# AIRI-Institute/nablaDFT

Measured on NVIDIA H100. Metric: molecules/sec (PaiNN E+F fwd+bwd), higher is better.
Workload: dtype f32

## Files before the change

nabladft_b200/csrc/painn_fused.cu:

```cuda
#include "painn_node.cuh"

#include "tc_pipe.cuh"

namespace {

constexpr int TILES_PER_LAYER = 22;

enum { T_UV = 0, T_UW, T_B1A, T_B1B, T_B2_0, T_B2_1, T_B2_2, T_A1, T_A2_0, T_A2_1, T_A2_2,
       T_B2T_0, T_B2T_1, T_B2T_2, T_B1AT, T_B1BT, T_UT_0, T_UT_1, T_A2T_0, T_A2T_1, T_A2T_2, T_A1T };

struct TileSrc { const float* p; int ld, row0, k0, trans, rows, kvalid; };

__device__ __forceinline__ TileSrc tile_src(const nb200_painn_weights& w, int idx) {
    const int L = w.n_layers;
    TileSrc s{nullptr, F, 0, 0, 0, 128, 128};
    if (idx >= L * TILES_PER_LAYER) {
        s.p = w.R1; s.ld = F;
        if (idx - L * TILES_PER_LAYER == 0) { s.rows = F / 2; } else { s.trans = 1; s.kvalid = F / 2; }
        return s;
    }
    const int l = idx / TILES_PER_LAYER, t = idx % TILES_PER_LAYER;
    const float* A1 = w.A1 + (size_t)l * F * F;
    const float* A2 = w.A2 + (size_t)l * 3 * F * F;
    const float* U = w.U + (size_t)l * 2 * F * F;
    const float* B1 = w.B1 + (size_t)l * F * 2 * F;
    const float* B2 = w.B2 + (size_t)l * 3 * F * F;
    switch (t) {
        case T_UV: s.p = U; break;
        case T_UW: s.p = U; s.row0 = F; break;
        case T_B1A: s.p = B1; s.ld = 2 * F; break;
        case T_B1B: s.p = B1; s.ld = 2 * F; s.k0 = F; break;
        case T_B2_0: case T_B2_1: case T_B2_2: s.p = B2; s.row0 = (t - T_B2_0) * F; break;
        case T_A1: s.p = A1; break;
        case T_A2_0: case T_A2_1: case T_A2_2: s.p = A2; s.row0 = (t - T_A2_0) * F; break;
        case T_B2T_0: case T_B2T_1: case T_B2T_2: s.p = B2; s.trans = 1; s.k0 = (t - T_B2T_0) * F; break;
        case T_B1AT: s.p = B1; s.ld = 2 * F; s.trans = 1; break;
        case T_B1BT: s.p = B1; s.ld = 2 * F; s.trans = 1; s.row0 = F; break;
        case T_UT_0: case T_UT_1: s.p = U; s.trans = 1; s.k0 = (t - T_UT_0) * F; break;
        case T_A2T_0: case T_A2T_1: case T_A2T_2: s.p = A2; s.trans = 1; s.k0 = (t - T_A2T_0) * F; break;
        default: s.p = A1; s.trans = 1; break;
    }
    return s;
}

__global__ void __launch_bounds__(256) k_prep_painn(nb200_painn_weights w, unsigned char* __restrict__ dst) {
    const int idx = blockIdx.x >> 2, st = blockIdx.x & 3;
    const TileSrc s = tile_src(w, idx);
    unsigned char* tile = dst + (size_t)idx * WTILE_BYTES;
#pragma unroll
    for (int i = 0; i < 4; ++i) {
        const int item = threadIdx.x + 256 * i;
        int kc, r;
        if (!s.trans) { kc = item & 7; r = item >> 3; } else { r = item & 127; kc = item >> 7; }
        const int k = st * 32 + kc * 4;
        float e[4];
#pragma unroll
        for (int j = 0; j < 4; ++j) {
            const bool ok = r < s.rows && k + j < s.kvalid;
            e[j] = !ok ? 0.f : !s.trans ? __ldg(s.p + (size_t)(s.row0 + r) * s.ld + s.k0 + k + j) : __ldg(s.p + (size_t)(s.k0 + k + j) * s.ld + s.row0 + r);
        }
        float4 hi, lo;
        split4(make_float4(e[0], e[1], e[2], e[3]), hi, lo);
        const int kk = 32 * st + 4 * kc;
        float* out_hi = reinterpret_cast<float*>(tile + (size_t)(kk / KSTAGE) * WST_BYTES + (size_t)((kk % KSTAGE) / 4) * WLBO) + r * 4;
        st4(out_hi, hi);
        st4(out_hi + (KSTAGE / 4) * WLBO / 4, lo);
    }
}

struct FwdParams {
    int xsplit;
    int n_atoms, do_upd, do_mlp, do_ro;
    const unsigned char* wt;
    int tile_upd, tile_mlp, tile_ro;
    const float *q_mid, *mu_mid, *d1, *d2;
    float *VW, *nrm, *dot, *g1pre, *y, *q_next, *mu_next;
    float eps;
    const float *q_mlp_in, *c1;
    float *h1pre, *xh;
    float* ro_pre;
};

__global__ void __launch_bounds__(NTHREADS, CTAS_PER_SM) k_node_fwd(const FwdParams P) {
    extern __shared__ __align__(1024) unsigned char smem[];
    __shared__ Prog prog;
    const int tid = threadIdx.x, warp = tid >> 5, lane = tid & 31;
    if (tid == 0) {
        prog.n = 0;
        if (P.do_upd) {
            for (int x = 0; x < 3; ++x) {
                prog_add(prog, P.tile_upd + T_UV, U_NEWX | U_FIRST | U_LAST);
                prog_add(prog, P.tile_upd + T_UW, U_FIRST | U_LAST | U_XLAST);
            }
            prog_add(prog, P.tile_upd + T_B1A, U_NEWX | U_FIRST | U_LAST | U_XLAST);
            prog_add(prog, P.tile_upd + T_B1B, U_NEWX | U_FIRST | U_LAST | U_XLAST);
            prog_add(prog, P.tile_upd + T_B2_1, U_NEWX | U_FIRST | U_LAST);
            prog_add(prog, P.tile_upd + T_B2_0, U_FIRST | U_LAST);
            prog_add(prog, P.tile_upd + T_B2_2, U_FIRST | U_LAST | U_XLAST);
        }
        if (P.do_mlp) {
            prog_add(prog, P.tile_mlp + T_A1, U_NEWX | U_FIRST | U_LAST | U_XLAST);
            prog_add(prog, P.tile_mlp + T_A2_0, U_NEWX | U_FIRST | U_LAST);
            prog_add(prog, P.tile_mlp + T_A2_1, U_FIRST | U_LAST);
            prog_add(prog, P.tile_mlp + T_A2_2, U_FIRST | U_LAST | U_XLAST);
        }
        if (P.do_ro) prog_add(prog, P.tile_ro, U_NEWX | U_FIRST | U_LAST | U_XLAST);
    }
    Ctx c = setup(smem, tid, P.xsplit);
    NF_PROF_DO(const long long tk0_ = clock64(); c.t_last = tk0_;)
#define NF_BASE 0

    if (warp >= WARP_ISSUE) {
        run_issuer(c, prog, P.wt);
        NF_PROF_DO(if (warp == WARP_ISSUE && lane == 0) { atomicAdd(&g_nf_prof[0], (unsigned long long)(clock64() - tk0_)); atomicAdd(&g_nf_prof[1], (unsigned long long)c.w_x);
                   atomicAdd(&g_nf_prof[2], (unsigned long long)c.w_buf); atomicAdd(&g_nf_prof[3], (unsigned long long)c.w_full); })
    } else {
        const int N = P.n_atoms, A0 = blockIdx.x * NT;
        const int fl = 32 * (warp & 3) + lane;
        const int n0 = CPT * (warp >> 2);
        const bool isE = role_epi(warp), isL = role_load(warp);
        const int ltid = load_tid(tid);
#define NF_LOAD(...) do { if (isL) load_x(c, ltid, __VA_ARGS__); else ++c.xg; } while (0)
        if (P.do_upd) {
#pragma unroll 1
            for (int x = 0; x < 3; ++x) {
                NF_LOAD([&](int r, int kc) { return A0 + r < N ? ldg4(P.mu_mid + (size_t)(A0 + r) * (3 * F) + x * F + 4 * kc) : f4(0.f); });
                NF_MARK(0);
#pragma unroll 1
                for (int half = 0; half < 2 && isE; ++half) {
                    drain(c, warp);
                    NF_MARK(1);
                    epi_chunks(c, warp, [&](int cb, float (&v)[16]) {
                        float* dst = P.VW + (size_t)(A0 + n0 + 16 * cb) * (6 * F) + x * 2 * F + half * F + fl;
#pragma unroll
                        for (int j = 0; j < 16; ++j)
                            if (A0 + n0 + 16 * cb + j < N) dst[(size_t)j * (6 * F)] = v[j];
                    });
                    NF_MARK(21);
                }
            }
            NF_MARK(2);
            if (isE) dep_signal(c, 0);
            NF_LOAD([&](int r, int kc) { return A0 + r < N ? ldg4(P.q_mid + (size_t)(A0 + r) * F + 4 * kc) : f4(0.f); });
            NF_MARK(3);
            if (isL) {
                dep_wait(c, 0);
                const int kc = ltid & 31, w = ltid >> 5;
#pragma unroll 1
                for (int it0 = 0; it0 < RPT; it0 += 2) {
                    float4 V[2][3], Wv[2][3];
#pragma unroll
                    for (int b = 0; b < 2; ++b) {
                        const int a = A0 + w + NLOAD * (it0 + b);
                        const float* vv = P.VW + (size_t)min(a, N - 1) * (6 * F) + 4 * kc;
#pragma unroll
                        for (int x = 0; x < 3; ++x) { V[b][x] = ld4(vv + x * 2 * F); Wv[b][x] = ld4(vv + x * 2 * F + F); }
                    }
#pragma unroll
                    for (int b = 0; b < 2; ++b) {
                        const int a = A0 + w + NLOAD * (it0 + b);
                        if (a < N) {
                            float4 sq = V[b][0] * V[b][0]; fma4(sq, V[b][1], V[b][1]); fma4(sq, V[b][2], V[b][2]);
                            float4 dt = f4(0.f); fma4(dt, V[b][0], Wv[b][0]); fma4(dt, V[b][1], Wv[b][1]); fma4(dt, V[b][2], Wv[b][2]);
                            st4(P.nrm + (size_t)a * F + 4 * kc, make_float4(sqrtf(sq.x + P.eps), sqrtf(sq.y + P.eps), sqrtf(sq.z + P.eps), sqrtf(sq.w + P.eps)));
                            st4(P.dot + (size_t)a * F + 4 * kc, dt);
                        }
                    }
                }
            }
            NF_MARK(4);
            if (isL) dep_signal(c, 1);
            NF_LOAD([&](int r, int kc) { return A0 + r < N ? ld4(P.nrm + (size_t)(A0 + r) * F + 4 * kc) : f4(0.f); });
            NF_MARK(5);
            if (isE) drain(c, warp);
            NF_MARK(6);
            NF_MARK(7);
            if (!isE) ++c.xg;
            else {
                drain(c, warp, 1);
                NF_MARK(8);
                const float b = __ldg(P.d1 + fl);
                const XPut xp(c, fl);
                epi_chunks(c, warp, [&](int cb, float (&v)[16]) {
#pragma unroll
                    for (int j = 0; j < 16; ++j) xp.put(n0 + 16 * cb + j, A0 + n0 + 16 * cb + j < N ? siluf_(v[j] + b) : 0.f);
                });
                xp.done(c);
                epi_chunks(c, warp, [&](int cb, float (&v)[16]) {
                    float* g = P.g1pre + (size_t)(A0 + n0 + 16 * cb) * F + fl;
#pragma unroll
                    for (int j = 0; j < 16; ++j)
                        if (A0 + n0 + 16 * cb + j < N) g[(size_t)j * F] = v[j] + b;
                });
            }
            NF_MARK(9);
            if (isE) {
                drain(c, warp);
                NF_MARK(10);
                const float b = __ldg(P.d2 + F + fl);
#pragma unroll 1
                for (int cb = 0; cb < CPT / 8; ++cb) {
                    float v16[16];
                    stage_ld16(c, warp, cb >> 1, v16);
                    float tw[8][3], tm[8][3];
#pragma unroll
                    for (int jj = 0; jj < 8; ++jj) {
                        const int a = min(A0 + n0 + 8 * cb + jj, N - 1);
                        const float* vw = P.VW + (size_t)a * (6 * F) + F + fl;
                        const float* mm = P.mu_mid + (size_t)a * (3 * F) + fl;
#pragma unroll
                        for (int x = 0; x < 3; ++x) { tw[jj][x] = vw[x * 2 * F]; tm[jj][x] = __ldg(mm + x * F); }
                    }
#pragma unroll
                    for (int jj = 0; jj < 8; ++jj) {
                        const int a = A0 + n0 + 8 * cb + jj;
                        if (a < N) {
                            const float y1 = ((cb & 1) ? v16[8 + jj] : v16[jj]) + b;
                            P.y[(size_t)a * (3 * F) + F + fl] = y1;
                            float* mo = P.mu_next + (size_t)a * (3 * F) + fl;
#pragma unroll
                            for (int x = 0; x < 3; ++x) mo[x * F] = fmaf(y1, tw[jj][x], tm[jj][x]);
                        }
                    }
                }
            }
            NF_MARK(11);
            if (isE) {
                drain(c, warp);
                NF_MARK(12);
                const float b = __ldg(P.d2 + fl);
                epi_chunks(c, warp, [&](int cb, float (&v)[16]) {
                    float t[16];
#pragma unroll
                    for (int j = 0; j < 16; ++j) t[j] = __ldg(P.q_mid + (size_t)min(A0 + n0 + 16 * cb + j, N - 1) * F + fl);
#pragma unroll
                    for (int j = 0; j < 16; ++j) {
                        const int a = A0 + n0 + 16 * cb + j;
                        if (a < N) {
                            const float y0 = v[j] + b;
                            P.y[(size_t)a * (3 * F) + fl] = y0;
                            P.q_next[(size_t)a * F + fl] = t[j] + y0;
                        }
                    }
                });
            }
            NF_MARK(13);
            if (!isE) ++c.xg;
            else {
                dep_wait(c, 1);
                drain(c, warp);
                NF_MARK(14);
                const float b = __ldg(P.d2 + 2 * F + fl);
                const XPut xp(c, fl);
                epi_chunks(c, warp, [&](int cb, float (&v)[16]) {
                    float tq[16], td[16];
#pragma unroll
                    for (int j = 0; j < 16; ++j) {
                        const size_t a = (size_t)min(A0 + n0 + 16 * cb + j, N - 1);
                        tq[j] = P.q_next[a * F + fl];
                        td[j] = P.dot[a * F + fl];
                    }
#pragma unroll
                    for (int j = 0; j < 16; ++j) {
                        const int a = A0 + n0 + 16 * cb + j;
                        float qn = 0.f;
                        if (a < N) {
                            qn = fmaf(v[j] + b, td[j], tq[j]);
                            P.q_next[(size_t)a * F + fl] = qn;
                        }
                        xp.put(n0 + 16 * cb + j, qn);
                    }
                });
                xp.done(c);
                epi_chunks(c, warp, [&](int cb, float (&v)[16]) {
#pragma unroll
                    for (int j = 0; j < 16; ++j)
                        if (A0 + n0 + 16 * cb + j < N) P.y[(size_t)(A0 + n0 + 16 * cb + j) * (3 * F) + 2 * F + fl] = v[j] + b;
                });
            }
        } else {
            NF_LOAD([&](int r, int kc) { return A0 + r < N ? ldg4(P.q_mlp_in + (size_t)(A0 + r) * F + 4 * kc) : f4(0.f); });
        }
        NF_MARK(15);
        if (P.do_mlp && !isE) ++c.xg;
        if (P.do_mlp && isE) {
            {
                drain(c, warp);
                NF_MARK(16);
                const float b = __ldg(P.c1 + fl);
                const XPut xp(c, fl);
                epi_chunks(c, warp, [&](int cb, float (&v)[16]) {
#pragma unroll
                    for (int j = 0; j < 16; ++j) xp.put(n0 + 16 * cb + j, siluf_(v[j] + b));
                });
                xp.done(c);
                epi_chunks(c, warp, [&](int cb, float (&v)[16]) {
#pragma unroll
                    for (int j = 0; j < 16; ++j)
                        if (A0 + n0 + 16 * cb + j < N) P.h1pre[(size_t)(A0 + n0 + 16 * cb + j) * F + fl] = v[j] + b;
                });
            }
            NF_MARK(17);
#pragma unroll 1
            for (int ct = 0; ct < 3; ++ct) {
                drain(c, warp);
                NF_MARK(18);
                epi_chunks(c, warp, [&](int cb, float (&v)[16]) {
                    float* dst = P.xh + (size_t)(A0 + n0 + 16 * cb) * (3 * F) + ct * F + fl;
#pragma unroll
                    for (int j = 0; j < 16; ++j)
                        if (A0 + n0 + 16 * cb + j < N) dst[(size_t)j * (3 * F)] = v[j];
                });
            }
        }
        NF_MARK(19);
        if (P.do_ro && isE) {
            drain(c, warp);
            epi_chunks(c, warp, [&](int cb, float (&v)[16]) {
                if (fl < F / 2) {
                    float* dst = P.ro_pre + (size_t)(A0 + n0 + 16 * cb) * (F / 2) + fl;
#pragma unroll
                    for (int j = 0; j < 16; ++j)
                        if (A0 + n0 + 16 * cb + j < N) dst[(size_t)j * (F / 2)] = v[j];
                }
            });
        }
#undef NF_LOAD
    }
    NF_MARK(20);
#undef NF_BASE
    NF_PROF_DO(if (tid == 0) { atomicAdd(&g_nf_prof[4], (unsigned long long)(clock64() - tk0_)); atomicAdd(&g_nf_prof[5], (unsigned long long)c.w_acc);
                            atomicAdd(&g_nf_prof[6], (unsigned long long)c.w_xfree); atomicAdd(&g_nf_prof[7], 1ull); })
}

struct BwdParams {
    int xsplit;
    int n_atoms, do_mlp, do_ro, do_upd;
    const unsigned char* wt;
    int tile_mlp, tile_ro, tile_upd;
    float *gq_a, *gq_b, *cur, *gn, *gdot;
    const float *g_xh, *h1pre, *dot;
    const float *ro_pre, *R2;
    const float *y, *VW, *nrm, *g1pre;
};

__global__ void __launch_bounds__(NTHREADS, CTAS_PER_SM) k_node_bwd(const BwdParams P) {
    extern __shared__ __align__(1024) unsigned char smem[];
    __shared__ Prog prog;
    const int tid = threadIdx.x, warp = tid >> 5, lane = tid & 31;
    if (tid == 0) {
        prog.n = 0;
        if (P.do_mlp) {
            prog_add(prog, P.tile_mlp + T_A2T_0, U_NEWX | U_FIRST | U_XLAST);
            prog_add(prog, P.tile_mlp + T_A2T_1, U_NEWX | U_XLAST);
            prog_add(prog, P.tile_mlp + T_A2T_2, U_NEWX | U_XLAST | U_LAST);
            prog_add(prog, P.tile_mlp + T_A1T, U_NEWX | U_FIRST | U_LAST | U_XLAST);
        } else if (P.do_ro) {
            prog_add(prog, P.tile_ro, U_NEWX | U_FIRST | U_LAST | U_XLAST);
        }
        if (P.do_upd) {
            prog_add(prog, P.tile_upd + T_B2T_0, U_NEWX | U_FIRST | U_XLAST);
            prog_add(prog, P.tile_upd + T_B2T_1, U_NEWX | U_XLAST);
            prog_add(prog, P.tile_upd + T_B2T_2, U_NEWX | U_XLAST | U_LAST);
            prog_add(prog, P.tile_upd + T_B1AT, U_NEWX | U_FIRST | U_LAST);
            prog_add(prog, P.tile_upd + T_B1BT, U_FIRST | U_LAST | U_XLAST);
            for (int x = 0; x < 3; ++x) {
                prog_add(prog, P.tile_upd + T_UT_0, U_NEWX | U_FIRST | U_XLAST);
                prog_add(prog, P.tile_upd + T_UT_1, U_NEWX | U_XLAST | U_LAST);
            }
        }
    }
    Ctx c = setup(smem, tid, P.xsplit);
    NF_PROF_DO(const long long tk0_ = clock64();)

    if (warp >= WARP_ISSUE) {
        run_issuer(c, prog, P.wt);
        NF_PROF_DO(if (warp == WARP_ISSUE && lane == 0) { atomicAdd(&g_nf_prof[8], (unsigned long long)(clock64() - tk0_)); atomicAdd(&g_nf_prof[9], (unsigned long long)c.w_x);
                   atomicAdd(&g_nf_prof[10], (unsigned long long)c.w_buf); atomicAdd(&g_nf_prof[11], (unsigned long long)c.w_full); })
    } else {
        const int N = P.n_atoms, A0 = blockIdx.x * NT;
        const int fl = 32 * (warp & 3) + lane;
        const int n0 = CPT * (warp >> 2);
        const bool isE = role_epi(warp), isL = role_load(warp);
        const int ltid = load_tid(tid);
#define NF_LOAD(...) do { if (isL) load_x(c, ltid, __VA_ARGS__); else ++c.xg; } while (0)
        if (P.do_mlp) {
#pragma unroll 1
            for (int ck = 0; ck < 3; ++ck)
                NF_LOAD([&](int r, int kc) { return A0 + r < N ? ldg4(P.g_xh + (size_t)(A0 + r) * (3 * F) + ck * F + 4 * kc) : f4(0.f); });
            if (!isE) ++c.xg;
            else {
                drain(c, warp);
                const XPut xp(c, fl);
                epi_chunks(c, warp, [&](int cb, float (&v)[16]) {
                    float t[16];
#pragma unroll
                    for (int j = 0; j < 16; ++j) t[j] = __ldg(P.h1pre + (size_t)min(A0 + n0 + 16 * cb + j, N - 1) * F + fl);
#pragma unroll
                    for (int j = 0; j < 16; ++j) xp.put(n0 + 16 * cb + j, A0 + n0 + 16 * cb + j < N ? v[j] * dsiluf_(t[j]) : 0.f);
                });
                xp.done(c);
            }
        } else if (P.do_ro) {
            NF_LOAD([&](int r, int kc) {
                if (A0 + r >= N || kc >= F / 8) return f4(0.f);
                const float4 p = ldg4(P.ro_pre + (size_t)(A0 + r) * (F / 2) + 4 * kc), w2 = ldg4(P.R2 + 4 * kc);
                return make_float4(w2.x * dsiluf_(p.x), w2.y * dsiluf_(p.y), w2.z * dsiluf_(p.z), w2.w * dsiluf_(p.w));
            });
        }
        if ((P.do_mlp || P.do_ro) && isE) {
            drain(c, warp);
            epi_chunks(c, warp, [&](int cb, float (&v)[16]) {
                float t[16], ty[16];
#pragma unroll
                for (int j = 0; j < 16; ++j) {
                    const size_t a = (size_t)min(A0 + n0 + 16 * cb + j, N - 1);
                    t[j] = P.do_mlp ? P.gq_a[a * F + fl] : 0.f;
                    ty[j] = P.do_upd ? __ldg(P.y + a * (3 * F) + 2 * F + fl) : 0.f;
                }
#pragma unroll
                for (int j = 0; j < 16; ++j) {
                    const int a = A0 + n0 + 16 * cb + j;
                    if (a < N) {
                        const float g = t[j] + v[j];
                        P.gq_b[(size_t)a * F + fl] = g;
                        if (P.do_upd) P.gdot[(size_t)a * F + fl] = g * ty[j];
                    }
                }
            });
        }
        if (P.do_upd) {
            if (isE) dep_signal(c, 0);
            if (isL) dep_wait(c, 0);
            NF_LOAD([&](int r, int kc) { return A0 + r < N ? ld4(P.gq_b + (size_t)(A0 + r) * F + 4 * kc) : f4(0.f); });
            NF_LOAD([&](int r, int kc) {
                if (A0 + r >= N) return f4(0.f);
                const float* vw = P.VW + (size_t)(A0 + r) * (6 * F) + F + 4 * kc;
                const float* gm = P.cur + (size_t)(A0 + r) * (3 * F) + 4 * kc;
                float4 sacc = f4(0.f);
#pragma unroll
                for (int x = 0; x < 3; ++x) fma4(sacc, ld4(gm + x * F), ldg4(vw + x * 2 * F));
                return sacc;
            });
            NF_LOAD([&](int r, int kc) {
                return A0 + r < N ? ld4(P.gq_b + (size_t)(A0 + r) * F + 4 * kc) * ldg4(P.dot + (size_t)(A0 + r) * F + 4 * kc) : f4(0.f);
            });
            if (!isE) ++c.xg;
            else {
                drain(c, warp);
                const XPut xp(c, fl);
                epi_chunks(c, warp, [&](int cb, float (&v)[16]) {
                    float t[16];
#pragma unroll
                    for (int j = 0; j < 16; ++j) t[j] = __ldg(P.g1pre + (size_t)min(A0 + n0 + 16 * cb + j, N - 1) * F + fl);
#pragma unroll
                    for (int j = 0; j < 16; ++j) xp.put(n0 + 16 * cb + j, A0 + n0 + 16 * cb + j < N ? v[j] * dsiluf_(t[j]) : 0.f);
                });
                xp.done(c);
            }
            if (isE) {
                drain(c, warp);
                epi_chunks(c, warp, [&](int cb, float (&v)[16]) {
                    float t[16];
#pragma unroll
                    for (int j = 0; j < 16; ++j) t[j] = P.gq_b[(size_t)min(A0 + n0 + 16 * cb + j, N - 1) * F + fl];
#pragma unroll
                    for (int j = 0; j < 16; ++j)
                        if (A0 + n0 + 16 * cb + j < N) P.gq_a[(size_t)(A0 + n0 + 16 * cb + j) * F + fl] = t[j] + v[j];
                });
            }
            if (isE) {
                drain(c, warp);
                epi_chunks(c, warp, [&](int cb, float (&v)[16]) {
                    float t[16];
#pragma unroll
                    for (int j = 0; j < 16; ++j) t[j] = __ldg(P.nrm + (size_t)min(A0 + n0 + 16 * cb + j, N - 1) * F + fl);
#pragma unroll
                    for (int j = 0; j < 16; ++j)
                        if (A0 + n0 + 16 * cb + j < N) P.gn[(size_t)(A0 + n0 + 16 * cb + j) * F + fl] = v[j] / t[j];
                });
            }
            if (isE) dep_signal(c, 1);
            if (isL) dep_wait(c, 1);
#pragma unroll 1
            for (int x = 0; x < 3; ++x) {
                NF_LOAD([&](int r, int kc) {
                    if (A0 + r >= N) return f4(0.f);
                    const size_t a = (size_t)(A0 + r);
                    float4 o = ld4(P.gdot + a * F + 4 * kc) * ldg4(P.VW + a * (6 * F) + x * 2 * F + F + 4 * kc);
                    fma4(o, ld4(P.gn + a * F + 4 * kc), ldg4(P.VW + a * (6 * F) + x * 2 * F + 4 * kc));
                    return o;
                });
                NF_LOAD([&](int r, int kc) {
                    if (A0 + r >= N) return f4(0.f);
                    const size_t a = (size_t)(A0 + r);
                    float4 o = ld4(P.cur + a * (3 * F) + x * F + 4 * kc) * ldg4(P.y + a * (3 * F) + F + 4 * kc);
                    fma4(o, ld4(P.gdot + a * F + 4 * kc), ldg4(P.VW + a * (6 * F) + x * 2 * F + 4 * kc));
                    return o;
                });
                if (isE) {
                drain(c, warp);
                epi_chunks(c, warp, [&](int cb, float (&v)[16]) {
                    float t[16];
#pragma unroll
                    for (int j = 0; j < 16; ++j) t[j] = P.cur[(size_t)min(A0 + n0 + 16 * cb + j, N - 1) * (3 * F) + x * F + fl];
#pragma unroll
                    for (int j = 0; j < 16; ++j)
                        if (A0 + n0 + 16 * cb + j < N) P.cur[(size_t)(A0 + n0 + 16 * cb + j) * (3 * F) + x * F + fl] = t[j] + v[j];
                });
                }
            }
        }
#undef NF_LOAD
    }
    NF_PROF_DO(if (tid == 0) { atomicAdd(&g_nf_prof[12], (unsigned long long)(clock64() - tk0_)); atomicAdd(&g_nf_prof[13], (unsigned long long)c.w_acc);
                            atomicAdd(&g_nf_prof[14], (unsigned long long)c.w_xfree); atomicAdd(&g_nf_prof[15], 1ull); })
}

template <class K>
int set_smem(K kernel) {
    return cudaFuncSetAttribute(kernel, cudaFuncAttributeMaxDynamicSharedMemorySize, SMEM_TOTAL) == cudaSuccess ? NB200_OK : nb_check_launch();
}

}

#ifdef NF_PROF
extern "C" int nb200_debug_nf_prof(unsigned long long* out16, int reset) {
    if (cudaMemcpyFromSymbol(out16, g_nf_prof, sizeof(unsigned long long) * 16) != cudaSuccess) return -1;
    if (reset) { unsigned long long z[16] = {0}; cudaMemcpyToSymbol(g_nf_prof, z, sizeof(z)); }
    return 0;
}
extern "C" int nb200_debug_nf_phase(unsigned long long* out64, int reset) {
    if (cudaMemcpyFromSymbol(out64, g_nf_phase, sizeof(unsigned long long) * 64) != cudaSuccess) return -1;
    if (reset) { unsigned long long z[64] = {0}; cudaMemcpyToSymbol(g_nf_phase, z, sizeof(z)); }
    return 0;
}
#endif

int64_t nb_fused_wtile_bytes(int n_layers) { return (int64_t)(n_layers * TILES_PER_LAYER + 2) * WTILE_BYTES; }

int nb_fused_prep(const nb200_painn_weights* w, void* wtiles, cudaStream_t s) {
    const int n_tiles = w->n_layers * TILES_PER_LAYER + 2;
    k_prep_painn<<<n_tiles * 4, 256, 0, s>>>(*w, static_cast<unsigned char*>(wtiles));
    return nb_check_launch();
}

static int nf_xsplit() {
    static const int on = [] { const char* e = getenv("NB200_NF_XSPLIT"); return (e && e[0] == '1') ? 1 : 0; }();
    return on;
}

int nb_fused_node_fwd(const NbFusedFwd& a, cudaStream_t s) {
    static bool attr = false;
    if (!attr) { if (set_smem(k_node_fwd) != NB200_OK) return NB200_ECUDA; attr = true; }
    FwdParams P{};
    P.xsplit = nf_xsplit();
    P.n_atoms = a.n_atoms; P.do_upd = a.layer_upd >= 0; P.do_mlp = a.layer_mlp >= 0; P.do_ro = a.readout;
    P.wt = static_cast<const unsigned char*>(a.wtiles);
    P.tile_upd = a.layer_upd * TILES_PER_LAYER; P.tile_mlp = a.layer_mlp * TILES_PER_LAYER; P.tile_ro = a.n_layers * TILES_PER_LAYER;
    P.q_mid = a.q_mid; P.mu_mid = a.mu_mid; P.d1 = a.d1; P.d2 = a.d2; P.VW = a.VW; P.nrm = a.nrm; P.dot = a.dot; P.g1pre = a.g1pre; P.y = a.y;
    P.q_next = a.q_next; P.mu_next = a.mu_next; P.eps = a.eps; P.q_mlp_in = a.q_mlp_in; P.c1 = a.c1; P.h1pre = a.h1pre; P.xh = a.xh;
    P.ro_pre = a.ro_pre;
    if (a.n_atoms <= 0) return NB200_OK;
    k_node_fwd<<<(a.n_atoms + NT - 1) / NT, NTHREADS, SMEM_TOTAL, s>>>(P);
    return nb_check_launch();
}

int nb_fused_node_bwd(const NbFusedBwd& a, cudaStream_t s) {
    static bool attr = false;
    if (!attr) { if (set_smem(k_node_bwd) != NB200_OK) return NB200_ECUDA; attr = true; }
    BwdParams P{};
    P.xsplit = nf_xsplit();
    P.n_atoms = a.n_atoms; P.do_mlp = a.layer_mlp >= 0; P.do_ro = a.readout; P.do_upd = a.layer_upd >= 0;
    P.wt = static_cast<const unsigned char*>(a.wtiles);
    P.tile_mlp = a.layer_mlp * TILES_PER_LAYER; P.tile_ro = a.n_layers * TILES_PER_LAYER + 1; P.tile_upd = a.layer_upd * TILES_PER_LAYER;
    P.gq_a = a.gq_a; P.gq_b = a.gq_b; P.cur = a.cur; P.gn = a.gn; P.gdot = a.gdot; P.dot = a.dot; P.g_xh = a.g_xh; P.h1pre = a.h1pre; P.ro_pre = a.ro_pre; P.R2 = a.R2;
    P.y = a.y; P.VW = a.VW; P.nrm = a.nrm; P.g1pre = a.g1pre;
    if (a.n_atoms <= 0) return NB200_OK;
    k_node_bwd<<<(a.n_atoms + NT - 1) / NT, NTHREADS, SMEM_TOTAL, s>>>(P);
    return nb_check_launch();
}
```

nabladft_b200/csrc/tc_pipe.cuh:

```cuda
#pragma once
#include "common.cuh"
#include "wgmma.cuh"

namespace {


constexpr int F = NB_F;
constexpr int NT = 64, KSTAGE = 32, W_STAGES = 3, NWORK = 8, CTAS_PER_SM = 1;
constexpr int XLBO = NT * 16 + 16;
constexpr int XLBOF = XLBO / 4;
constexpr int X_BYTES = 32 * XLBO;
constexpr int WLBO = 128 * 16;
constexpr int WST_BYTES = 2 * (KSTAGE / 4) * WLBO;
constexpr int STAGES_PER_TILE = 128 / KSTAGE;
constexpr int WTILE_BYTES = STAGES_PER_TILE * WST_BYTES;
constexpr int SROW = NT + 4;
constexpr int STAGE_BYTES = 128 * SROW * 4;
constexpr int SMEM_BARS = 2 * X_BYTES + W_STAGES * WST_BYTES + STAGE_BYTES;
constexpr int SMEM_TOTAL = SMEM_BARS + 256;
static_assert(SMEM_TOTAL <= 227 * 1024, "shared memory of one CTA");
#ifdef NF_TWO_GROUPS
constexpr int NEPI = NWORK / 2, NLOAD = NWORK / 2;
#else
constexpr int NEPI = NWORK, NLOAD = NWORK;
#endif
constexpr int CPT = NT / (NEPI / 4);
constexpr int RPT = NT / NLOAD;
constexpr int WARP_ISSUE = NWORK;
constexpr int NTHREADS = 32 * (NWORK + 8);
static_assert(NWORK % 4 == 0, "the MMA warpgroups must start on a warpgroup boundary");
enum { U_NEWX = 1, U_FIRST = 2, U_LAST = 4, U_XLAST = 8 };
#ifdef NF_PROF
__device__ unsigned long long g_nf_prof[16];
__device__ unsigned long long g_nf_phase[64];
#define NF_PROF_DO(...) __VA_ARGS__
#define NF_MARK(i) do { if (tid == 0) { const long long now_ = clock64(); atomicAdd(&g_nf_phase[NF_BASE + (i)], (unsigned long long)(now_ - c.t_last)); c.t_last = now_; } } while (0)
#else
#define NF_PROF_DO(...)
#define NF_MARK(i)
#endif

struct Prog {
    int n;
    uint16_t tile[24];
    uint8_t flag[24];
};

__device__ __forceinline__ uint32_t s_u32(const void* p) { return (uint32_t)__cvta_generic_to_shared(p); }
__device__ __forceinline__ void mbar_init(uint64_t* bar, uint32_t count) {
    asm volatile("mbarrier.init.shared::cta.b64 [%0], %1;" ::"r"(s_u32(bar)), "r"(count) : "memory");
}
__device__ __forceinline__ void mbar_wait(uint64_t* bar, uint32_t parity) {
    asm volatile(
        "{\n.reg .pred P1;\nLAB_WAIT:\nmbarrier.try_wait.parity.shared::cta.b64 P1, [%0], %1;\n@P1 bra DONE;\nbra LAB_WAIT;\nDONE:\n}\n" ::"r"(
            s_u32(bar)),
        "r"(parity)
        : "memory");
}
__device__ __forceinline__ void mbar_arrive(uint64_t* bar) { asm volatile("mbarrier.arrive.shared::cta.b64 _, [%0];" ::"r"(s_u32(bar)) : "memory"); }
__device__ __forceinline__ void mbar_expect_tx(uint64_t* bar, uint32_t bytes) {
    asm volatile("mbarrier.arrive.expect_tx.shared::cta.b64 _, [%0], %1;" ::"r"(s_u32(bar)), "r"(bytes) : "memory");
}
__device__ __forceinline__ void bulk_g2s(void* dst, const void* src, uint32_t bytes, uint64_t* bar) {
    asm volatile("cp.async.bulk.shared::cluster.global.mbarrier::complete_tx::bytes [%0], [%1], %2, [%3];" ::"r"(s_u32(dst)), "l"(src), "r"(bytes),
                 "r"(s_u32(bar))
                 : "memory");
}
__device__ __forceinline__ float tf32_rn(float x) {
    uint32_t r;
    asm("cvt.rna.tf32.f32 %0, %1;" : "=r"(r) : "f"(x));
    return __uint_as_float(r);
}
__device__ __forceinline__ void split_tf32(float x, float& hi, float& lo) {
    hi = tf32_rn(x);
    lo = tf32_rn(x - hi);
}
__device__ __forceinline__ void split4(const float4 v, float4& hi, float4& lo) {
    split_tf32(v.x, hi.x, lo.x); split_tf32(v.y, hi.y, lo.y); split_tf32(v.z, hi.z, lo.z); split_tf32(v.w, hi.w, lo.w);
}
__device__ __forceinline__ void work_barrier() { asm volatile("bar.sync 1, %0;" ::"n"(32 * NWORK) : "memory"); }
__device__ __forceinline__ float4 ld4(const float* p) { return *reinterpret_cast<const float4*>(p); }

struct Ctx {
    float *x_hi, *x_lo;
    unsigned char* ring;
    float* stage;
    uint64_t *full, *empty, *x_ready, *x_free, *acc_full, *stage_free, *dep;
    uint64_t *x_ready2, *x_free2;
    int xsplit = 0;
    int xg = 0;
    int o = 0;
    NF_PROF_DO(long long w_acc = 0, w_xfree = 0, w_x = 0, w_buf = 0, w_full = 0, t_last = 0;)
};

template <class FlagFn, class TileFn>
__device__ __forceinline__ void run_issuer_t(Ctx& c, int n_units, FlagFn flags_of, TileFn tile_of, const unsigned char* wt, int spt = STAGES_PER_TILE) {
    const int wl = ((threadIdx.x >> 5) - WARP_ISSUE) & 3, h = ((threadIdx.x >> 5) - WARP_ISSUE) >> 2, lane = threadIdx.x & 31;
    float corr[NT / 2], main0[NT / 2], main1[NT / 2];
    const uint32_t x_hi0 = s_u32(c.x_hi), x_lo0 = s_u32(c.x_lo);
    const int n_q = n_units * spt;
    const bool leader = threadIdx.x == 32 * WARP_ISSUE;
    int q = 0, pending = -1;
    auto release = [&](uint64_t* bar) { if (lane == 0) mbar_arrive(bar); };
    auto copy = [&](int qq) {
        if (!leader || qq >= n_q) return;
        const int slot = qq % W_STAGES;
        mbar_expect_tx(c.full + slot, WST_BYTES);
        bulk_g2s(c.ring + slot * WST_BYTES, wt + (size_t)tile_of(qq / spt) * WTILE_BYTES + (size_t)(qq % spt) * WST_BYTES, WST_BYTES, c.full + slot);
    };
    auto free_stage = [&](int pq) {
        const int slot = pq % W_STAGES;
        release(c.empty + slot);
        if (leader) { mbar_wait(c.empty + slot, (uint32_t)((pq / W_STAGES) & 1)); copy(pq + W_STAGES); }
    };
    for (int qq = 0; qq < W_STAGES; ++qq) copy(qq);
#pragma unroll 1
    for (int u = 0; u < n_units; ++u) {
        const int fl = flags_of(u);
        const bool newx = (fl & U_NEWX) != 0;
        if (newx) { NF_PROF_DO(const long long t0_ = clock64();) mbar_wait(c.x_ready, (uint32_t)(c.xg & 1)); ++c.xg; NF_PROF_DO(c.w_x += clock64() - t0_;) }
        if (fl & U_FIRST) {
#pragma unroll
            for (int i = 0; i < NT / 2; ++i) { corr[i] = 0.f; main0[i] = 0.f; main1[i] = 0.f; }
        }
#pragma unroll 1
        for (int st = 0; st < spt; ++st, ++q) {
            const int slot = q % W_STAGES;
            if (c.xsplit && newx && st == STAGES_PER_TILE / 2) {
                NF_PROF_DO(const long long t0_ = clock64();)
                mbar_wait(c.x_ready2, (uint32_t)((c.xg - 1) & 1));
                NF_PROF_DO(c.w_x += clock64() - t0_;)
            }
            NF_PROF_DO(const long long t1_ = clock64();)
            mbar_wait(c.full + slot, (uint32_t)((q / W_STAGES) & 1));
            NF_PROF_DO(c.w_full += clock64() - t1_;)
            const uint32_t wh = s_u32(c.ring + slot * WST_BYTES), wlo = wh + (KSTAGE / 4) * WLBO;
            const uint32_t xoff = (uint32_t)(st * (KSTAGE / 4) * XLBO);
            wgmma_fence();
#pragma unroll
            for (int ks = 0; ks < KSTAGE / 8; ++ks) {
                const uint64_t dxh = gmma_desc(x_hi0 + xoff + 2 * ks * XLBO, XLBO, 128), dxl = gmma_desc(x_lo0 + xoff + 2 * ks * XLBO, XLBO, 128);
                const uint64_t dwh = gmma_desc(wh + 2 * ks * WLBO + h * 1024, WLBO, 128), dwl = gmma_desc(wlo + 2 * ks * WLBO + h * 1024, WLBO, 128);
                wgmma_tf32_n64(corr, dwl, dxh);
                wgmma_tf32_n64(corr, dwh, dxl);
                if (ks & 1) wgmma_tf32_n64(main1, dwh, dxh);
                else wgmma_tf32_n64(main0, dwh, dxh);
            }
            wgmma_commit();
            wgmma_wait<1>();
            if (pending >= 0) free_stage(pending);
            pending = q;
            if (c.xsplit && (fl & U_XLAST) && st == STAGES_PER_TILE / 2 - 1) {
                wgmma_wait<0>();
                free_stage(pending); pending = -1;
                release(c.x_free);
            }
        }
        wgmma_wait<0>();
        if (pending >= 0) { free_stage(pending); pending = -1; }
        if (fl & U_XLAST) {
            if (!c.xsplit) release(c.x_free);
            else { if (spt < STAGES_PER_TILE / 2) release(c.x_free); release(c.x_free2); }
        }
        if (fl & U_LAST) {
            if (c.o > 0) { NF_PROF_DO(const long long t2_ = clock64();) mbar_wait(c.stage_free, (uint32_t)((c.o - 1) & 1)); NF_PROF_DO(c.w_buf += clock64() - t2_;) }
            const int f = 64 * h + 16 * wl + (lane >> 2);
#pragma unroll
            for (int j = 0; j < NT / 8; ++j) {
                const int n = 8 * j + 2 * (lane & 3);
                *reinterpret_cast<float2*>(c.stage + f * SROW + n) = make_float2(corr[4 * j] + (main0[4 * j] + main1[4 * j]), corr[4 * j + 1] + (main0[4 * j + 1] + main1[4 * j + 1]));
                *reinterpret_cast<float2*>(c.stage + (f + 8) * SROW + n) = make_float2(corr[4 * j + 2] + (main0[4 * j + 2] + main1[4 * j + 2]), corr[4 * j + 3] + (main0[4 * j + 3] + main1[4 * j + 3]));
            }
            mbar_arrive(c.acc_full);
            ++c.o;
        }
    }
}
__device__ __forceinline__ void run_issuer(Ctx& c, const Prog& prog, const unsigned char* wt) {
    run_issuer_t(c, prog.n, [&](int u) { return (int)prog.flag[u]; }, [&](int u) { return (int)prog.tile[u]; }, wt);
}

template <class Fn>
__device__ __forceinline__ void load_x(Ctx& c, int wtid, Fn f) {
    if (c.xsplit) {
        const int lane = wtid & 31, wrp = wtid >> 5, half = wrp >= NLOAD / 2 ? 1 : 0, w8 = wrp - half * (NLOAD / 2);
        const int kc = (lane & 15) + 16 * half, rsub = lane >> 4;
        constexpr int ITEMS = (NT * 16) / (32 * (NLOAD / 2));
        static_assert(ITEMS * 32 * (NLOAD / 2) == NT * 16 && ITEMS <= 16, "load_x xsplit mapping");
        float4 t[ITEMS];
#pragma unroll
        for (int it = 0; it < ITEMS; ++it) t[it] = f(2 * (w8 + (NLOAD / 2) * it) + rsub, kc);
        NF_PROF_DO(const long long t0_ = clock64();)
        if (c.xg > 0) mbar_wait(half ? c.x_free2 : c.x_free, (uint32_t)((c.xg - 1) & 1));
        NF_PROF_DO(c.w_xfree += clock64() - t0_;)
#pragma unroll
        for (int it = 0; it < ITEMS; ++it) {
            const int r = 2 * (w8 + (NLOAD / 2) * it) + rsub;
            float4 hi, lo;
            split4(t[it], hi, lo);
            st4(c.x_hi + kc * XLBOF + r * 4, hi);
            st4(c.x_lo + kc * XLBOF + r * 4, lo);
        }
        asm volatile("fence.proxy.async.shared::cta;" ::: "memory");
        mbar_arrive(half ? c.x_ready2 : c.x_ready);
        ++c.xg;
        return;
    }
    const int kc = wtid & 31, w = wtid >> 5;
#pragma unroll 1
    for (int h = 0; h < RPT / 8; ++h) {
        float4 t[8];
#pragma unroll
        for (int it = 0; it < 8; ++it) t[it] = f(w + NLOAD * (8 * h + it), kc);
        NF_PROF_DO(const long long t0_ = clock64();)
        if (c.xg > 0) mbar_wait(c.x_free, (uint32_t)((c.xg - 1) & 1));
        NF_PROF_DO(c.w_xfree += clock64() - t0_;)
#pragma unroll
        for (int it = 0; it < 8; ++it) {
            const int r = w + NLOAD * (8 * h + it);
            float4 hi, lo;
            split4(t[it], hi, lo);
            st4(c.x_hi + kc * XLBOF + r * 4, hi);
            st4(c.x_lo + kc * XLBOF + r * 4, lo);
        }
    }
    asm volatile("fence.proxy.async.shared::cta;" ::: "memory");
    mbar_arrive(c.x_ready);
    ++c.xg;
}

struct XPut {
    float *hi, *lo;
    bool second;
    __device__ __forceinline__ XPut(const Ctx& c, int k) {
        second = c.xsplit && k >= 64;
        if (c.xg > 0) mbar_wait(second ? c.x_free2 : c.x_free, (uint32_t)((c.xg - 1) & 1));
        hi = c.x_hi + (k >> 2) * XLBOF + (k & 3);
        lo = c.x_lo + (k >> 2) * XLBOF + (k & 3);
    }
    __device__ __forceinline__ void put(int n, float v) const {
        float h, l;
        split_tf32(v, h, l);
        hi[n * 4] = h;
        lo[n * 4] = l;
    }
    __device__ __forceinline__ void done(Ctx& c) const {
        asm volatile("fence.proxy.async.shared::cta;" ::: "memory");
        mbar_arrive(second ? c.x_ready2 : c.x_ready);
        ++c.xg;
    }
};

__device__ __forceinline__ void drain(Ctx& c, int warp, int add_stage = 0) {
    NF_PROF_DO(const long long t0_ = clock64();)
    float* mine = c.stage + (32 * (warp & 3) + (threadIdx.x & 31)) * SROW + (warp >> 2) * CPT;
    if (add_stage) {
        float4 keep[CPT / 4];
#pragma unroll
        for (int i = 0; i < CPT / 4; ++i) keep[i] = reinterpret_cast<const float4*>(mine)[i];
        if (c.o > 0) mbar_arrive(c.stage_free);
        mbar_wait(c.acc_full, (uint32_t)(c.o & 1));
#pragma unroll
        for (int i = 0; i < CPT / 4; ++i) reinterpret_cast<float4*>(mine)[i] = reinterpret_cast<const float4*>(mine)[i] + keep[i];
    } else {
        if (c.o > 0) mbar_arrive(c.stage_free);
        mbar_wait(c.acc_full, (uint32_t)(c.o & 1));
    }
    NF_PROF_DO(c.w_acc += clock64() - t0_;)
    ++c.o;
}

__device__ __forceinline__ void stage_ld16(const Ctx& c, int warp, int cb, float (&v)[16]) {
    const float4* src = reinterpret_cast<const float4*>(c.stage + (32 * (warp & 3) + (threadIdx.x & 31)) * SROW + (warp >> 2) * CPT + cb * 16);
#pragma unroll
    for (int i = 0; i < 4; ++i) {
        const float4 t = src[i];
        v[4 * i] = t.x; v[4 * i + 1] = t.y; v[4 * i + 2] = t.z; v[4 * i + 3] = t.w;
    }
}

__device__ __forceinline__ void prog_add(Prog& p, int tile, int flags) {
    p.tile[p.n] = (uint16_t)tile;
    p.flag[p.n] = (uint8_t)flags;
    ++p.n;
}

__device__ __forceinline__ Ctx setup(unsigned char* smem, int tid, int xsplit = 0) {
    Ctx c;
    c.xsplit = xsplit;
    c.x_hi = reinterpret_cast<float*>(smem);
    c.x_lo = reinterpret_cast<float*>(smem + X_BYTES);
    c.ring = smem + 2 * X_BYTES;
    c.stage = reinterpret_cast<float*>(smem + 2 * X_BYTES + W_STAGES * WST_BYTES);
    uint64_t* bars = reinterpret_cast<uint64_t*>(smem + SMEM_BARS);
    c.full = bars; c.empty = bars + W_STAGES; c.x_ready = bars + 2 * W_STAGES; c.x_free = c.x_ready + 1; c.acc_full = c.x_ready + 2;
    c.stage_free = c.x_ready + 3;
    c.dep = c.x_ready + 6;
    c.x_ready2 = c.x_ready + 11; c.x_free2 = c.x_ready + 12;
    if (tid == 0) {
        for (int s = 0; s < W_STAGES; ++s) { mbar_init(c.full + s, 1); mbar_init(c.empty + s, 8); }
        mbar_init(c.x_ready, xsplit ? 16 * NLOAD : 32 * NLOAD);
        mbar_init(c.x_free, 8);
        mbar_init(c.x_ready2, 16 * NLOAD);
        mbar_init(c.x_free2, 8);
        mbar_init(c.acc_full, 256);
        mbar_init(c.stage_free, 32 * NEPI);
        for (int b = 0; b < 4; ++b) mbar_init(c.dep + b, 32 * NLOAD);
        asm volatile("fence.mbarrier_init.release.cluster;" ::: "memory");
    }
    __syncthreads();
    return c;
}

__device__ __forceinline__ bool role_epi(int warp) { return warp < NEPI; }
#ifdef NF_TWO_GROUPS
__device__ __forceinline__ bool role_load(int warp) { return warp >= NEPI && warp < NEPI + NLOAD; }
__device__ __forceinline__ int load_tid(int tid) { return tid - 32 * NEPI; }
#else
__device__ __forceinline__ bool role_load(int warp) { return warp < NLOAD; }
__device__ __forceinline__ int load_tid(int tid) { return tid; }
#endif
__device__ __forceinline__ void dep_signal(const Ctx& c, int k) {
#ifdef NF_TWO_GROUPS
    mbar_arrive(c.dep + k);
#else
    (void)c; (void)k;
    work_barrier();
#endif
}
__device__ __forceinline__ void dep_wait(const Ctx& c, int k) {
#ifdef NF_TWO_GROUPS
    mbar_wait(c.dep + k, 0u);
#else
    (void)c; (void)k;
#endif
}

template <class Body>
__device__ __forceinline__ void epi_chunks(const Ctx& c, int warp, Body body) {
#pragma unroll 1
    for (int cb = 0; cb < CPT / 16; ++cb) {
        float v[16];
        stage_ld16(c, warp, cb, v);
        body(cb, v);
    }
}


}
```

Baseline: 64500.

## Split backward node kernel into two independent atom-half pipelines

The backward kernel now runs a two-halves schedule. Each issuer warpgroup computes all 128 output features for its own 32-atom half using n32 wgmma, and gets its own x-ready, x-free, accumulator and stage barriers, so the two halves advance without waiting on each other. Weight-ring refills are triggered by a shared atomic counter instead of a leader waiting on an empty mbarrier. The final update loop is software-pipelined so the epilogue for component x-1 overlaps the loads for x. This adds a more complex synchronisation scheme and drops the xsplit option from the backward pass.

```diff
diff --git a/nabladft_b200/csrc/painn_fused.cu b/nabladft_b200/csrc/painn_fused.cu
--- a/nabladft_b200/csrc/painn_fused.cu
+++ b/nabladft_b200/csrc/painn_fused.cu
@@ -111,8 +111,9 @@
 #define NF_BASE 0
 
     if (warp >= WARP_ISSUE) {
-        run_issuer(c, prog, P.wt);
-        NF_PROF_DO(if (warp == WARP_ISSUE && lane == 0) { atomicAdd(&g_nf_prof[0], (unsigned long long)(clock64() - tk0_)); atomicAdd(&g_nf_prof[1], (unsigned long long)c.w_x);
+        run_issuer<false>(c, prog, P.wt);
+        NF_PROF_DO(if ((warp - WARP_ISSUE) % 4 == 0 && lane == 0) {
+                   atomicAdd(&g_nf_prof[0], (unsigned long long)(clock64() - tk0_)); atomicAdd(&g_nf_prof[1], (unsigned long long)c.w_x);
                    atomicAdd(&g_nf_prof[2], (unsigned long long)c.w_buf); atomicAdd(&g_nf_prof[3], (unsigned long long)c.w_full); })
     } else {
         const int N = P.n_atoms, A0 = blockIdx.x * NT;
@@ -329,12 +330,12 @@
     }
     NF_MARK(20);
 #undef NF_BASE
-    NF_PROF_DO(if (tid == 0) { atomicAdd(&g_nf_prof[4], (unsigned long long)(clock64() - tk0_)); atomicAdd(&g_nf_prof[5], (unsigned long long)c.w_acc);
+    NF_PROF_DO(if (warp < WARP_ISSUE && tid % 128 == 0) {
+                   atomicAdd(&g_nf_prof[4], (unsigned long long)(clock64() - tk0_)); atomicAdd(&g_nf_prof[5], (unsigned long long)c.w_acc);
                             atomicAdd(&g_nf_prof[6], (unsigned long long)c.w_xfree); atomicAdd(&g_nf_prof[7], 1ull); })
 }
 
 struct BwdParams {
-    int xsplit;
     int n_atoms, do_mlp, do_ro, do_upd;
     const unsigned char* wt;
     int tile_mlp, tile_ro, tile_upd;
@@ -370,12 +371,13 @@
             }
         }
     }
-    Ctx c = setup(smem, tid, P.xsplit);
+    Ctx c = setup(smem, tid, 0, 1);
     NF_PROF_DO(const long long tk0_ = clock64();)
 
     if (warp >= WARP_ISSUE) {
-        run_issuer(c, prog, P.wt);
-        NF_PROF_DO(if (warp == WARP_ISSUE && lane == 0) { atomicAdd(&g_nf_prof[8], (unsigned long long)(clock64() - tk0_)); atomicAdd(&g_nf_prof[9], (unsigned long long)c.w_x);
+        run_issuer<true>(c, prog, P.wt);
+        NF_PROF_DO(if ((warp - WARP_ISSUE) % 4 == 0 && lane == 0) {
+                   atomicAdd(&g_nf_prof[8], (unsigned long long)(clock64() - tk0_)); atomicAdd(&g_nf_prof[9], (unsigned long long)c.w_x);
                    atomicAdd(&g_nf_prof[10], (unsigned long long)c.w_buf); atomicAdd(&g_nf_prof[11], (unsigned long long)c.w_full); })
     } else {
         const int N = P.n_atoms, A0 = blockIdx.x * NT;
@@ -483,37 +485,41 @@
             if (isE) dep_signal(c, 1);
             if (isL) dep_wait(c, 1);
 #pragma unroll 1
-            for (int x = 0; x < 3; ++x) {
-                NF_LOAD([&](int r, int kc) {
-                    if (A0 + r >= N) return f4(0.f);
-                    const size_t a = (size_t)(A0 + r);
-                    float4 o = ld4(P.gdot + a * F + 4 * kc) * ldg4(P.VW + a * (6 * F) + x * 2 * F + F + 4 * kc);
-                    fma4(o, ld4(P.gn + a * F + 4 * kc), ldg4(P.VW + a * (6 * F) + x * 2 * F + 4 * kc));
-                    return o;
-                });
-                NF_LOAD([&](int r, int kc) {
-                    if (A0 + r >= N) return f4(0.f);
-                    const size_t a = (size_t)(A0 + r);
-                    float4 o = ld4(P.cur + a * (3 * F) + x * F + 4 * kc) * ldg4(P.y + a * (3 * F) + F + 4 * kc);
-                    fma4(o, ld4(P.gdot + a * F + 4 * kc), ldg4(P.VW + a * (6 * F) + x * 2 * F + 4 * kc));
-                    return o;
-                });
-                if (isE) {
-                drain(c, warp);
-                epi_chunks(c, warp, [&](int cb, float (&v)[16]) {
-                    float t[16];
-#pragma unroll
-                    for (int j = 0; j < 16; ++j) t[j] = P.cur[(size_t)min(A0 + n0 + 16 * cb + j, N - 1) * (3 * F) + x * F + fl];
-#pragma unroll
-                    for (int j = 0; j < 16; ++j)
-                        if (A0 + n0 + 16 * cb + j < N) P.cur[(size_t)(A0 + n0 + 16 * cb + j) * (3 * F) + x * F + fl] = t[j] + v[j];
-                });
-                }
+            for (int x = 0; x <= 3; ++x) {
+                if (x < 3)
+                    NF_LOAD([&](int r, int kc) {
+                        if (A0 + r >= N) return f4(0.f);
+                        const size_t a = (size_t)(A0 + r);
+                        float4 o = ld4(P.gdot + a * F + 4 * kc) * ldg4(P.VW + a * (6 * F) + x * 2 * F + F + 4 * kc);
+                        fma4(o, ld4(P.gn + a * F + 4 * kc), ldg4(P.VW + a * (6 * F) + x * 2 * F + 4 * kc));
+                        return o;
+                    });
+                if (x > 0 && isE) {
+                    const int xe = x - 1;
+                    drain(c, warp);
+                    epi_chunks(c, warp, [&](int cb, float (&v)[16]) {
+                        float t[16];
+#pragma unroll
+                        for (int j = 0; j < 16; ++j) t[j] = P.cur[(size_t)min(A0 + n0 + 16 * cb + j, N - 1) * (3 * F) + xe * F + fl];
+#pragma unroll
+                        for (int j = 0; j < 16; ++j)
+                            if (A0 + n0 + 16 * cb + j < N) P.cur[(size_t)(A0 + n0 + 16 * cb + j) * (3 * F) + xe * F + fl] = t[j] + v[j];
+                    });
+                }
+                if (x < 3)
+                    NF_LOAD([&](int r, int kc) {
+                        if (A0 + r >= N) return f4(0.f);
+                        const size_t a = (size_t)(A0 + r);
+                        float4 o = ld4(P.cur + a * (3 * F) + x * F + 4 * kc) * ldg4(P.y + a * (3 * F) + F + 4 * kc);
+                        fma4(o, ld4(P.gdot + a * F + 4 * kc), ldg4(P.VW + a * (6 * F) + x * 2 * F + 4 * kc));
+                        return o;
+                    });
             }
         }
 #undef NF_LOAD
     }
-    NF_PROF_DO(if (tid == 0) { atomicAdd(&g_nf_prof[12], (unsigned long long)(clock64() - tk0_)); atomicAdd(&g_nf_prof[13], (unsigned long long)c.w_acc);
+    NF_PROF_DO(if (warp < WARP_ISSUE && tid % 128 == 0) {
+                   atomicAdd(&g_nf_prof[12], (unsigned long long)(clock64() - tk0_)); atomicAdd(&g_nf_prof[13], (unsigned long long)c.w_acc);
                             atomicAdd(&g_nf_prof[14], (unsigned long long)c.w_xfree); atomicAdd(&g_nf_prof[15], 1ull); })
 }
 
@@ -570,7 +576,6 @@
     static bool attr = false;
     if (!attr) { if (set_smem(k_node_bwd) != NB200_OK) return NB200_ECUDA; attr = true; }
     BwdParams P{};
-    P.xsplit = nf_xsplit();
     P.n_atoms = a.n_atoms; P.do_mlp = a.layer_mlp >= 0; P.do_ro = a.readout; P.do_upd = a.layer_upd >= 0;
     P.wt = static_cast<const unsigned char*>(a.wtiles);
     P.tile_mlp = a.layer_mlp * TILES_PER_LAYER; P.tile_ro = a.n_layers * TILES_PER_LAYER + 1; P.tile_upd = a.layer_upd * TILES_PER_LAYER;
diff --git a/nabladft_b200/csrc/tc_pipe.cuh b/nabladft_b200/csrc/tc_pipe.cuh
--- a/nabladft_b200/csrc/tc_pipe.cuh
+++ b/nabladft_b200/csrc/tc_pipe.cuh
@@ -78,7 +78,11 @@
 __device__ __forceinline__ void split4(const float4 v, float4& hi, float4& lo) {
     split_tf32(v.x, hi.x, lo.x); split_tf32(v.y, hi.y, lo.y); split_tf32(v.z, hi.z, lo.z); split_tf32(v.w, hi.w, lo.w);
 }
-__device__ __forceinline__ void work_barrier() { asm volatile("bar.sync 1, %0;" ::"n"(32 * NWORK) : "memory"); }
+__device__ __forceinline__ uint32_t atom_add_acq_rel(uint32_t* p, uint32_t v) {
+    uint32_t old;
+    asm volatile("atom.acq_rel.cta.shared::cta.add.u32 %0, [%1], %2;" : "=r"(old) : "r"(s_u32(p)), "r"(v) : "memory");
+    return old;
+}
 __device__ __forceinline__ float4 ld4(const float* p) { return *reinterpret_cast<const float4*>(p); }
 
 struct Ctx {
@@ -86,34 +90,43 @@
     unsigned char* ring;
     float* stage;
     uint64_t *full, *empty, *x_ready, *x_free, *acc_full, *stage_free, *dep;
+    uint32_t* ring_cnt;
     uint64_t *x_ready2, *x_free2;
     int xsplit = 0;
+    int halves = 0;
+    int hf = 0;
     int xg = 0;
     int o = 0;
     NF_PROF_DO(long long w_acc = 0, w_xfree = 0, w_x = 0, w_buf = 0, w_full = 0, t_last = 0;)
 };
 
-template <class FlagFn, class TileFn>
+template <bool Halves = false, class FlagFn, class TileFn>
 __device__ __forceinline__ void run_issuer_t(Ctx& c, int n_units, FlagFn flags_of, TileFn tile_of, const unsigned char* wt, int spt = STAGES_PER_TILE) {
+    static_assert(!Halves || NEPI == NWORK, "the two-halves schedule uses one worker group per half");
     const int wl = ((threadIdx.x >> 5) - WARP_ISSUE) & 3, h = ((threadIdx.x >> 5) - WARP_ISSUE) >> 2, lane = threadIdx.x & 31;
     float corr[NT / 2], main0[NT / 2], main1[NT / 2];
     const uint32_t x_hi0 = s_u32(c.x_hi), x_lo0 = s_u32(c.x_lo);
     const int n_q = n_units * spt;
-    const bool leader = threadIdx.x == 32 * WARP_ISSUE;
     int q = 0, pending = -1;
     auto release = [&](uint64_t* bar) { if (lane == 0) mbar_arrive(bar); };
+    const bool leader = threadIdx.x == 32 * WARP_ISSUE;
     auto copy = [&](int qq) {
-        if (!leader || qq >= n_q) return;
+        if (qq >= n_q) return;
         const int slot = qq % W_STAGES;
         mbar_expect_tx(c.full + slot, WST_BYTES);
         bulk_g2s(c.ring + slot * WST_BYTES, wt + (size_t)tile_of(qq / spt) * WTILE_BYTES + (size_t)(qq % spt) * WST_BYTES, WST_BYTES, c.full + slot);
     };
     auto free_stage = [&](int pq) {
         const int slot = pq % W_STAGES;
-        release(c.empty + slot);
-        if (leader) { mbar_wait(c.empty + slot, (uint32_t)((pq / W_STAGES) & 1)); copy(pq + W_STAGES); }
+        if constexpr (Halves) {
+            if (lane == 0 && atom_add_acq_rel(c.ring_cnt + slot, 1u) % 8 == 7) copy(pq + W_STAGES);
+        } else {
+            release(c.empty + slot);
+            if (leader) { mbar_wait(c.empty + slot, (uint32_t)((pq / W_STAGES) & 1)); copy(pq + W_STAGES); }
+        }
     };
-    for (int qq = 0; qq < W_STAGES; ++qq) copy(qq);
+    if (leader)
+        for (int qq = 0; qq < W_STAGES; ++qq) copy(qq);
 #pragma unroll 1
     for (int u = 0; u < n_units; ++u) {
         const int fl = flags_of(u);
@@ -139,12 +152,26 @@
             wgmma_fence();
 #pragma unroll
             for (int ks = 0; ks < KSTAGE / 8; ++ks) {
-                const uint64_t dxh = gmma_desc(x_hi0 + xoff + 2 * ks * XLBO, XLBO, 128), dxl = gmma_desc(x_lo0 + xoff + 2 * ks * XLBO, XLBO, 128);
-                const uint64_t dwh = gmma_desc(wh + 2 * ks * WLBO + h * 1024, WLBO, 128), dwl = gmma_desc(wlo + 2 * ks * WLBO + h * 1024, WLBO, 128);
-                wgmma_tf32_n64(corr, dwl, dxh);
-                wgmma_tf32_n64(corr, dwh, dxl);
-                if (ks & 1) wgmma_tf32_n64(main1, dwh, dxh);
-                else wgmma_tf32_n64(main0, dwh, dxh);
+                if constexpr (Halves) {
+                    const uint32_t xo = xoff + 2 * ks * XLBO + h * 32 * 16;
+                    const uint64_t dxh = gmma_desc(x_hi0 + xo, XLBO, 128), dxl = gmma_desc(x_lo0 + xo, XLBO, 128);
+#pragma unroll
+                    for (int fb = 0; fb < 2; ++fb) {
+                        const uint64_t dwh = gmma_desc(wh + 2 * ks * WLBO + fb * 1024, WLBO, 128), dwl = gmma_desc(wlo + 2 * ks * WLBO + fb * 1024, WLBO, 128);
+                        float(&cf)[16] = *reinterpret_cast<float(*)[16]>(corr + 16 * fb);
+                        wgmma_tf32_n32(cf, dwl, dxh);
+                        wgmma_tf32_n32(cf, dwh, dxl);
+                        if (ks & 1) wgmma_tf32_n32(*reinterpret_cast<float(*)[16]>(main1 + 16 * fb), dwh, dxh);
+                        else wgmma_tf32_n32(*reinterpret_cast<float(*)[16]>(main0 + 16 * fb), dwh, dxh);
+                    }
+                } else {
+                    const uint64_t dxh = gmma_desc(x_hi0 + xoff + 2 * ks * XLBO, XLBO, 128), dxl = gmma_desc(x_lo0 + xoff + 2 * ks * XLBO, XLBO, 128);
+                    const uint64_t dwh = gmma_desc(wh + 2 * ks * WLBO + h * 1024, WLBO, 128), dwl = gmma_desc(wlo + 2 * ks * WLBO + h * 1024, WLBO, 128);
+                    wgmma_tf32_n64(corr, dwl, dxh);
+                    wgmma_tf32_n64(corr, dwh, dxl);
+                    if (ks & 1) wgmma_tf32_n64(main1, dwh, dxh);
+                    else wgmma_tf32_n64(main0, dwh, dxh);
+                }
             }
             wgmma_commit();
             wgmma_wait<1>();
@@ -164,10 +191,10 @@
         }
         if (fl & U_LAST) {
             if (c.o > 0) { NF_PROF_DO(const long long t2_ = clock64();) mbar_wait(c.stage_free, (uint32_t)((c.o - 1) & 1)); NF_PROF_DO(c.w_buf += clock64() - t2_;) }
-            const int f = 64 * h + 16 * wl + (lane >> 2);
 #pragma unroll
             for (int j = 0; j < NT / 8; ++j) {
-                const int n = 8 * j + 2 * (lane & 3);
+                const int f = (Halves ? 64 * (j >> 2) : 64 * h) + 16 * wl + (lane >> 2);
+                const int n = (Halves ? 32 * h + 8 * (j & 3) : 8 * j) + 2 * (lane & 3);
                 *reinterpret_cast<float2*>(c.stage + f * SROW + n) = make_float2(corr[4 * j] + (main0[4 * j] + main1[4 * j]), corr[4 * j + 1] + (main0[4 * j + 1] + main1[4 * j + 1]));
                 *reinterpret_cast<float2*>(c.stage + (f + 8) * SROW + n) = make_float2(corr[4 * j + 2] + (main0[4 * j + 2] + main1[4 * j + 2]), corr[4 * j + 3] + (main0[4 * j + 3] + main1[4 * j + 3]));
             }
@@ -176,8 +203,13 @@
         }
     }
 }
+template <bool Halves>
 __device__ __forceinline__ void run_issuer(Ctx& c, const Prog& prog, const unsigned char* wt) {
-    run_issuer_t(c, prog.n, [&](int u) { return (int)prog.flag[u]; }, [&](int u) { return (int)prog.tile[u]; }, wt);
+    run_issuer_t<Halves>(c, prog.n, [&](int u) { return (int)prog.flag[u]; }, [&](int u) { return (int)prog.tile[u]; }, wt);
+}
+
+__device__ __forceinline__ int x_row(const Ctx& c, int wtid, int i) {
+    return c.halves ? 32 * (wtid >> 7) + ((wtid >> 5) & 3) + 4 * i : (wtid >> 5) + NLOAD * i;
 }
 
 template <class Fn>
@@ -206,18 +238,18 @@
         ++c.xg;
         return;
     }
-    const int kc = wtid & 31, w = wtid >> 5;
+    const int kc = wtid & 31;
 #pragma unroll 1
     for (int h = 0; h < RPT / 8; ++h) {
         float4 t[8];
 #pragma unroll
-        for (int it = 0; it < 8; ++it) t[it] = f(w + NLOAD * (8 * h + it), kc);
+        for (int it = 0; it < 8; ++it) t[it] = f(x_row(c, wtid, 8 * h + it), kc);
         NF_PROF_DO(const long long t0_ = clock64();)
         if (c.xg > 0) mbar_wait(c.x_free, (uint32_t)((c.xg - 1) & 1));
         NF_PROF_DO(c.w_xfree += clock64() - t0_;)
 #pragma unroll
         for (int it = 0; it < 8; ++it) {
-            const int r = w + NLOAD * (8 * h + it);
+            const int r = x_row(c, wtid, 8 * h + it);
             float4 hi, lo;
             split4(t[it], hi, lo);
             st4(c.x_hi + kc * XLBOF + r * 4, hi);
@@ -285,27 +317,43 @@
     ++p.n;
 }
 
-__device__ __forceinline__ Ctx setup(unsigned char* smem, int tid, int xsplit = 0) {
+__device__ __forceinline__ Ctx setup(unsigned char* smem, int tid, int xsplit = 0, int halves = 0) {
     Ctx c;
     c.xsplit = xsplit;
+    c.halves = halves;
+    const int warp = tid >> 5;
+    c.hf = !halves ? 0 : warp >= WARP_ISSUE ? (warp - WARP_ISSUE) >> 2 : warp >> 2;
     c.x_hi = reinterpret_cast<float*>(smem);
     c.x_lo = reinterpret_cast<float*>(smem + X_BYTES);
     c.ring = smem + 2 * X_BYTES;
     c.stage = reinterpret_cast<float*>(smem + 2 * X_BYTES + W_STAGES * WST_BYTES);
     uint64_t* bars = reinterpret_cast<uint64_t*>(smem + SMEM_BARS);
-    c.full = bars; c.empty = bars + W_STAGES; c.x_ready = bars + 2 * W_STAGES; c.x_free = c.x_ready + 1; c.acc_full = c.x_ready + 2;
-    c.stage_free = c.x_ready + 3;
-    c.dep = c.x_ready + 6;
-    c.x_ready2 = c.x_ready + 11; c.x_free2 = c.x_ready + 12;
+    c.full = bars; c.empty = bars + W_STAGES;
+    c.ring_cnt = reinterpret_cast<uint32_t*>(bars + 2 * W_STAGES);
+    c.dep = bars + 2 * W_STAGES + 2;
+    uint64_t* hb = bars + 2 * W_STAGES + 6;
+    c.x_ready = hb + 6 * c.hf; c.x_free = c.x_ready + 1; c.acc_full = c.x_ready + 2; c.stage_free = c.x_ready + 3;
+    c.x_ready2 = c.x_ready + 4; c.x_free2 = c.x_ready + 5;
+    static_assert((2 * W_STAGES + 6 + 12) * 8 <= SMEM_TOTAL - SMEM_BARS, "barrier area");
     if (tid == 0) {
-        for (int s = 0; s < W_STAGES; ++s) { mbar_init(c.full + s, 1); mbar_init(c.empty + s, 8); }
-        mbar_init(c.x_ready, xsplit ? 16 * NLOAD : 32 * NLOAD);
-        mbar_init(c.x_free, 8);
-        mbar_init(c.x_ready2, 16 * NLOAD);
-        mbar_init(c.x_free2, 8);
-        mbar_init(c.acc_full, 256);
-        mbar_init(c.stage_free, 32 * NEPI);
+        for (int s = 0; s < W_STAGES; ++s) { mbar_init(c.full + s, 1); mbar_init(c.empty + s, 8); c.ring_cnt[s] = 0; }
         for (int b = 0; b < 4; ++b) mbar_init(c.dep + b, 32 * NLOAD);
+        for (int h = 0; h < (halves ? 2 : 1); ++h) {
+            uint64_t* x_ready = hb + 6 * h;
+            if (halves) {
+                mbar_init(x_ready, 128);
+                mbar_init(x_ready + 1, 4);
+                mbar_init(x_ready + 2, 128);
+                mbar_init(x_ready + 3, 128);
+            } else {
+                mbar_init(x_ready, xsplit ? 16 * NLOAD : 32 * NLOAD);
+                mbar_init(x_ready + 1, 8);
+                mbar_init(x_ready + 2, 256);
+                mbar_init(x_ready + 3, 32 * NEPI);
+                mbar_init(x_ready + 4, 16 * NLOAD);
+                mbar_init(x_ready + 5, 8);
+            }
+        }
         asm volatile("fence.mbarrier_init.release.cluster;" ::: "memory");
     }
     __syncthreads();
@@ -324,8 +372,9 @@
 #ifdef NF_TWO_GROUPS
     mbar_arrive(c.dep + k);
 #else
-    (void)c; (void)k;
-    work_barrier();
+    (void)k;
+    if (c.halves) asm volatile("bar.sync %0, 128;" ::"r"(2 + c.hf) : "memory");
+    else asm volatile("bar.sync 1, %0;" ::"n"(32 * NWORK) : "memory");
 #endif
 }
 __device__ __forceinline__ void dep_wait(const Ctx& c, int k) {
```

Result: faster. 65520 (median of 6 runs) (+1.6%).
